# RagnarGrootKoerkamp/astar-pairwise-aligner

Hardware: AMD Instinct MI355X
Metric: DP cell-updates/sec (GCUPS), full bit-parallel DP, 100kbp@5% div (higher is better)
Workload: dtype u32

## Files before the change

### astar-pairwise-aligner_amd/capi.py

```python
from __future__ import annotations

import ctypes as C
import os
from pathlib import Path

import numpy as np

from . import _build

U64P = C.POINTER(C.c_uint64)

EXPORTED_SYMBOLS = [
    "astarpa2_simple", "astarpa2_full", "astarpa", "astarpa_gcsh", "astarpa_free_cigar",
    "pa_last_error", "pa_device_count", "pa_set_device",
    "pa_bp_profile_build", "pa_bp_compute", "pa_bp_fill", "pa_search", "pa_search_trace",
    "pa_batch_create", "pa_batch_run", "pa_batch_stats", "pa_batch_shape", "pa_batch_destroy",
    "pa_batch_create_banded", "pa_batch_create_trace", "pa_batch_align", "pa_batch_align_view", "pa_batch_trace_fallbacks", "pa_params_batch_align",
    "pa_pairs_read", "pa_pairs_count", "pa_pairs_get", "pa_pairs_free", "pa_write_results_csv", "pa_align_file",
    "pa_align", "pa_batch_align_multi", "pa_batch_create_trace_params",
    "pa_bp_ctx_create", "pa_bp_ctx_compute", "pa_bp_ctx_fill", "pa_bp_ctx_destroy",
    "pa_batch_create_params", "pa_batch_pair_stats", "pa_runtime_hints", "pa_batch_align_multi_params", "pa_release_pools", "pa_align_file_params", "pa_batch_params_supported", "pa_alloc_cache_stats", "pa_free_cigars",
    "pa_batch_full_info", "pa_batch_rdv_stats", "pa_combine_stats", "pa_params_nw", "pa_params_simple", "pa_params_full", "pa_debug_gcsh_probe", "pa_debug_gcsh_matches", "pa_debug_strip", "pa_batch_window_retries", "pa_batch_window_retry_bytes",
    "pa_batch_slice_info", "pa_set_reference_cost_only",
    "pa_search_batch_create", "pa_search_batch_run", "pa_search_batch_rows", "pa_search_batch_trace", "pa_search_batch_info",
    "pa_search_batch_destroy",
    "pa_affine_batch_create", "pa_affine_batch_run", "pa_affine_batch_align", "pa_affine_batch_info", "pa_affine_batch_destroy",
]

_lib = None


class PaError(RuntimeError):
    pass


def load(build_if_stale: bool = True) -> C.CDLL:
    global _lib
    if _lib is not None:
        return _lib
    path = _build.LIB_PATH
    if os.environ.get("PA_LIB_PATH"):
        from pathlib import Path

        path, build_if_stale = Path(os.environ["PA_LIB_PATH"]).resolve(), False
    if build_if_stale and _build.is_stale():
        try:
            _build.build()
        except Exception as e:
            if not path.exists():
                raise PaError(f"cannot build {path.name}: {e}") from e
    if not path.exists():
        raise PaError(f"{path} is missing: run __graft_entry__.build() (hipcc --offload-arch=gfx950)")
    L = C.CDLL(str(path))
    L.pa_runtime_hints.restype = C.c_int
    if hasattr(L, "pa_set_reference_cost_only"):
        L.pa_set_reference_cost_only.argtypes = [C.c_int]
        L.pa_set_reference_cost_only.restype = None
    L.pa_release_pools.restype = None
    L.pa_alloc_cache_stats.argtypes = [C.POINTER(C.c_uint64)] * 3
    L.pa_free_cigars.argtypes = [C.c_void_p, C.c_size_t]
    L.pa_free_cigars.restype = None
    L.pa_batch_params_supported.argtypes = [C.c_void_p]
    L.pa_batch_params_supported.restype = C.c_int
    L.pa_alloc_cache_stats.restype = None
    L.pa_runtime_hints()
    vp, sz = C.c_void_p, C.c_size_t
    L.pa_last_error.restype = C.c_char_p
    L.pa_device_count.restype = C.c_int
    L.pa_set_device.argtypes = [C.c_int]
    L.pa_bp_profile_build.argtypes = [vp, sz, vp, sz, vp, vp]
    L.pa_bp_profile_build.restype = C.c_int
    L.pa_bp_compute.argtypes = [vp, sz, vp, sz, vp, vp, C.c_int]
    L.pa_bp_compute.restype = C.c_int32
    L.pa_bp_fill.argtypes = [vp, sz, vp, sz, vp, vp, vp]
    L.pa_bp_fill.restype = C.c_int32
    L.pa_search.argtypes = [vp, sz, vp, sz, C.c_float, vp]
    L.pa_search.restype = C.c_int
    L.pa_search_trace.argtypes = [vp, sz, vp, sz, C.c_float, sz, C.POINTER(vp), C.POINTER(vp), C.POINTER(sz)]
    L.pa_search_trace.restype = C.c_int
    L.pa_search_batch_create.argtypes = [vp, vp, sz, vp, vp, sz, vp, vp, sz, C.c_float]
    L.pa_search_batch_create.restype = vp
    L.pa_search_batch_run.argtypes = [vp, vp, vp, C.POINTER(C.c_float)]
    L.pa_search_batch_rows.argtypes = [vp, vp, vp]
    L.pa_search_batch_trace.argtypes = [vp, vp, vp, vp]
    L.pa_search_batch_info.argtypes = [vp] + [C.POINTER(C.c_double)] * 4
    L.pa_search_batch_info.restype = None
    L.pa_search_batch_destroy.argtypes = [vp]
    L.pa_affine_batch_create.argtypes = [vp, vp, vp, vp, sz, vp, C.c_int]
    L.pa_affine_batch_create.restype = vp
    L.pa_affine_batch_run.argtypes = [vp, vp, C.POINTER(C.c_float)]
    L.pa_affine_batch_align.argtypes = [vp, vp, vp, C.POINTER(C.c_float), C.POINTER(C.c_float)]
    L.pa_affine_batch_info.argtypes = [vp] + [C.POINTER(C.c_double)] * 5
    L.pa_affine_batch_info.restype = None
    L.pa_affine_batch_destroy.argtypes = [vp]
    L.pa_search_batch_destroy.restype = None
    L.pa_batch_create.argtypes = [vp, vp, vp, vp, sz]
    L.pa_batch_create.restype = vp
    L.pa_batch_run.argtypes = [vp, vp, C.POINTER(C.c_float)]
    L.pa_batch_run.restype = C.c_int
    L.pa_batch_stats.argtypes = [vp] + [C.POINTER(C.c_double)] * 4
    L.pa_batch_full_info.argtypes = [vp] + [C.POINTER(C.c_double)] * 4 + [C.POINTER(C.c_double)]
    L.pa_batch_full_info.restype = None
    L.pa_batch_rdv_stats.argtypes = [vp, C.POINTER(C.c_uint64)]
    L.pa_combine_stats.argtypes = [C.POINTER(C.c_uint64), C.POINTER(C.c_uint64)]
    L.pa_combine_stats.restype = None
    L.pa_batch_rdv_stats.restype = C.c_int
    L.pa_batch_shape.argtypes = [vp, C.POINTER(C.c_int), C.POINTER(C.c_int), C.POINTER(C.c_double)]
    L.pa_batch_slice_info.argtypes = [vp] + [C.POINTER(C.c_double)] * 5
    L.pa_batch_slice_info.restype = C.c_int
    L.pa_batch_destroy.argtypes = [vp]
    L.pa_batch_create_banded.argtypes = [vp, vp, vp, vp, sz, C.c_float]
    L.pa_batch_create_banded.restype = vp
    L.pa_batch_create_trace.argtypes = [vp, vp, vp, vp, sz]
    L.pa_batch_create_trace.restype = vp
    L.pa_bp_ctx_create.argtypes = [vp, sz, vp, sz]
    L.pa_bp_ctx_create.restype = vp
    L.pa_bp_ctx_compute.argtypes = [vp, C.c_int32, C.c_int32, sz, sz, vp, C.c_int, C.POINTER(C.c_int32)]
    L.pa_bp_ctx_compute.restype = C.c_int
    L.pa_bp_ctx_fill.argtypes = [vp, C.c_int32, C.c_int32, sz, sz, vp, vp, vp]
    L.pa_bp_ctx_fill.restype = C.c_int
    L.pa_bp_ctx_destroy.argtypes = [vp]
    L.pa_batch_create_trace_params.argtypes = [vp, vp, vp, vp, sz, vp]
    L.pa_batch_create_trace_params.restype = vp
    L.pa_batch_create_params.argtypes = [vp, vp, vp, vp, sz, vp]
    L.pa_batch_create_params.restype = vp
    L.pa_batch_pair_stats.argtypes = [vp, vp]
    L.pa_batch_pair_stats.restype = C.c_int
    L.pa_batch_align.argtypes = [vp, vp, vp, C.POINTER(C.c_float), C.POINTER(C.c_float)]
    L.pa_batch_align.restype = C.c_int
    L.pa_batch_align_view.argtypes = [vp, vp, vp, vp, C.POINTER(C.c_float), C.POINTER(C.c_float)]
    L.pa_batch_align_view.restype = C.c_int
    L.pa_batch_trace_fallbacks.argtypes = [vp]
    L.pa_batch_trace_fallbacks.restype = C.c_size_t
    L.pa_batch_window_retries.argtypes = [vp]
    L.pa_batch_window_retries.restype = C.c_size_t
    L.pa_pairs_read.argtypes = [C.c_char_p]
    L.pa_pairs_read.restype = vp
    L.pa_pairs_count.argtypes = [vp]
    L.pa_pairs_count.restype = sz
    L.pa_pairs_get.argtypes = [vp, sz, C.POINTER(vp), C.POINTER(sz), C.POINTER(vp), C.POINTER(sz)]
    L.pa_pairs_get.restype = C.c_int
    L.pa_pairs_free.argtypes = [vp]
    L.pa_write_results_csv.argtypes = [C.c_char_p, vp, vp, sz]
    L.pa_write_results_csv.restype = C.c_int
    L.pa_batch_align_multi.argtypes = [vp, vp, vp, vp, sz, C.POINTER(C.c_int), C.c_int, vp, vp]
    L.pa_batch_align_multi.restype = C.c_int
    L.pa_batch_align_multi_params.argtypes = [vp, vp, vp, vp, sz, C.POINTER(C.c_int), C.c_int, vp, vp, vp, vp]
    L.pa_batch_align_multi_params.restype = C.c_int
    L.pa_align_file.argtypes = [C.c_char_p, C.c_char_p, C.POINTER(sz)]
    L.pa_align_file.restype = C.c_int
    L.pa_align_file_params.argtypes = [C.c_char_p, C.c_char_p, vp, C.POINTER(sz)]
    L.pa_align_file_params.restype = C.c_int
    for name in ("astarpa2_simple", "astarpa2_full", "astarpa"):
        if hasattr(L, name):
            f = getattr(L, name)
            f.argtypes = [vp, sz, vp, sz, C.POINTER(vp), C.POINTER(sz)]
            f.restype = C.c_uint64
    if hasattr(L, "astarpa_gcsh"):
        L.astarpa_gcsh.argtypes = [vp, sz, vp, sz, sz, sz, C.c_bool, C.POINTER(vp), C.POINTER(sz)]
        L.astarpa_gcsh.restype = C.c_uint64
    if hasattr(L, "astarpa_free_cigar"):
        L.astarpa_free_cigar.argtypes = [vp]
    _lib = L
    return L


def last_error() -> str:
    return (load().pa_last_error() or b"").decode()


def _p(arr: np.ndarray):
    return arr.ctypes.data_as(C.c_void_p)


def _buf(b: bytes):
    return C.cast(C.c_char_p(b), C.c_void_p)
# ... 669 lines not shown
```

### astar-pairwise-aligner_amd/csrc/slice_kernel.hpp

```cpp
#pragma once
#include <hip/hip_runtime.h>
#include <stdint.h>

namespace pa {
namespace slice {

#ifndef PA_SLICE_CLOCK_TURNS
#define PA_SLICE_CLOCK_TURNS 15
#endif
#ifndef PA_SLICE_YIELD
#define PA_SLICE_YIELD 2
#endif
constexpr int kPad = 64;
constexpr int kErrSpin = 7;
constexpr uint32_t kSpinLimit = 1u << 22;

struct SliceGroup {
    uint64_t a_off;
    uint64_t b_off;
    uint64_t h_off;
    uint32_t h_stride;
    int32_t n;
    int32_t nstrips;
    int32_t npairs;
    uint32_t first_pos;
    uint32_t ev_first, ev_count;
    uint32_t pad_;
};
struct SliceEvent {
    int32_t col;
    uint32_t mask;
};
struct SliceJob {
    uint32_t group, strip;
};
struct SlicePair {
    uint64_t code_off, prof_off;
    int32_t n, m;
    uint32_t pair;
    uint32_t pad_;
};

typedef uint32_t pa_slice_u32x2 __attribute__((ext_vector_type(2)));
__device__ __forceinline__ uint32_t dpp_wave_shr1(uint32_t old_, uint32_t src) {
    return (uint32_t)__builtin_amdgcn_update_dpp((int)old_, (int)src, 0x138, 0xf, 0xf, false);
}
__device__ __forceinline__ uint32_t dpp_wave_rol1(uint32_t x) {
    return (uint32_t)__builtin_amdgcn_update_dpp((int)x, (int)x, 0x134, 0xf, 0xf, false);
}
__device__ __forceinline__ uint2 ld_boundary(const uint2* p) {
    const unsigned long long v = __hip_atomic_load((const unsigned long long*)p, __ATOMIC_RELAXED, __HIP_MEMORY_SCOPE_AGENT);
    return make_uint2((uint32_t)v, (uint32_t)(v >> 32));
}
__device__ __forceinline__ void st_boundary(uint2* p, uint32_t hp, uint32_t hm) {
    __hip_atomic_store((unsigned long long*)p, (unsigned long long)hp | ((unsigned long long)hm << 32), __ATOMIC_RELAXED, __HIP_MEMORY_SCOPE_AGENT);
}

#define PA_SLICE_ROW_PAIR(vpA, vmA, vpB, vmB, nb0A, nb1A, nb0B, nb1B, a0, a1, hpp, hmp, hpo, hmo)                                      \
    do {                                                                                                                                \
        uint32_t zA_, zB_, hmA_, hpA_;                                                                                                  \
        asm volatile(                                                                                                                   \
            "v_xor_b32 %[zA], %[a1_], %[nb1A_]\n\t"                                                                                     \
            "v_xor_b32 %[zB], %[a1_], %[nb1B_]\n\t"                                                                                     \
            "v_bitop3_b32 %[zA], %[a0_], %[nb0A_], %[zA] bitop3:0x28\n\t"                                                               \
            "v_bitop3_b32 %[zB], %[a0_], %[nb0B_], %[zB] bitop3:0x28\n\t"                                                               \
            "v_bitop3_b32 %[zA], %[zA], %[vmA_], %[hmp_] bitop3:0xfe\n\t"                                                               \
            "v_and_b32 %[hmA], %[zA], %[vpA_]\n\t"                                                                                      \
            "v_bitop3_b32 %[hpA], %[vmA_], %[zA], %[vpA_] bitop3:0xf1\n\t"                                                              \
            "v_bitop3_b32 %[zB], %[zB], %[vmB_], %[hmA] bitop3:0xfe\n\t"                                                                \
            "v_bitop3_b32 %[vpA_], %[hmp_], %[zA], %[hpp_] bitop3:0xf1\n\t"                                                             \
            "v_and_b32 %[hmB], %[zB], %[vpB_]\n\t"                                                                                      \
            "v_and_b32 %[vmA_], %[hpp_], %[zA]\n\t"                                                                                     \
            "v_bitop3_b32 %[hpB], %[vmB_], %[zB], %[vpB_] bitop3:0xf1\n\t"                                                              \
            "v_bitop3_b32 %[vpB_], %[hmA], %[zB], %[hpA] bitop3:0xf1\n\t"                                                               \
            "v_and_b32 %[vmB_], %[hpA], %[zB]"                                                                                          \
            : [zA] "=&v"(zA_), [zB] "=&v"(zB_), [hmA] "=&v"(hmA_), [hpA] "=&v"(hpA_), [hmB] "=&v"(hmo), [hpB] "=&v"(hpo),              \
              [vpA_] "+v"(vpA), [vmA_] "+v"(vmA), [vpB_] "+v"(vpB), [vmB_] "+v"(vmB)                                                    \
            : [a0_] "v"(a0), [a1_] "v"(a1), [nb0A_] "v"(nb0A), [nb1A_] "v"(nb1A), [nb0B_] "v"(nb0B), [nb1B_] "v"(nb1B), [hpp_] "v"(hpp), \
              [hmp_] "v"(hmp));                                                                                                         \
    } while (0)

template <int R>
__global__ __launch_bounds__(64, 2) void slice_kernel(const SliceJob* __restrict__ jobs, int njobs, const SliceGroup* __restrict__ groups,
                                                      const SliceEvent* __restrict__ events, const uint2* __restrict__ A, const uint2* __restrict__ B,
                                                      uint2* H, uint2* V, uint32_t* ticket_err, unsigned long long* dbg) {
    static_assert(R % 2 == 0, "rows are stepped in pairs");
    const int lane = (int)threadIdx.x;
    const uint32_t wave_slot = (uint32_t)__builtin_amdgcn_s_getreg((4 - 1) << 11 | 4) & 15u;
    for (;;) {
        uint32_t tk = 0;
        if (lane == 0) tk = atomicAdd(ticket_err, 1u);
        tk = (uint32_t)__builtin_amdgcn_readfirstlane((int)tk);
        if (tk >= (uint32_t)njobs) break;
        const SliceJob job = jobs[tk];
        const SliceGroup grp = groups[job.group];
        const unsigned long long t_job0 = dbg ? __builtin_amdgcn_s_memrealtime() : 0ull;
        unsigned long long t_parked = 0, n_parks = 0;
        [[maybe_unused]] bool waited_before = false;
        [[maybe_unused]] int slack = 0;
        const int s = (int)job.strip, n = grp.n;
        const bool has_in = s > 0, has_out = s + 1 < grp.nstrips;
        const uint2* Ag = A + grp.a_off + kPad;
        const size_t row0 = grp.b_off + ((size_t)s * 64 + (size_t)lane) * R;
        const uint2* Hin = H + grp.h_off + (size_t)(has_in ? s - 1 : 0) * grp.h_stride + kPad;
        uint2* Hout = H + grp.h_off + (size_t)(has_out ? s : 0) * grp.h_stride + kPad;
        const SliceEvent* ev = events + grp.ev_first;
        uint32_t nb0[R], nb1[R], vp[R], vm[R];
#pragma unroll
        for (int i = 0; i < R; ++i) {
            const uint2 b = B[row0 + i];
            nb0[i] = b.x;
            nb1[i] = b.y;
            vp[i] = ~0u;
            vm[i] = 0u;
        }
        constexpr int kWaitStep = 8;
        uint32_t o_hp = 0, o_hm = 0, o_a0 = 0, o_a1 = 0;
        uint32_t ev_i = 0;
        int ev_col = ev[0].col;
        const int nchunks = (n + 63 + 63) / 64;
        const __amdgpu_buffer_rsrc_t hrs = __builtin_amdgcn_make_buffer_rsrc((void*)Hout, 0, (int)((uint32_t)n * 8u), 0x00020000);
        unsigned long long nA = 0, nH = ~0ull;
        uint2 kA = Ag[lane], kH = make_uint2(~0u, 0u);
        if (has_in) kH = ld_boundary(Hin + lane);
        __builtin_amdgcn_s_waitcnt(0);
        for (int q = 0; q < nchunks; ++q) {
#if PA_SLICE_CLOCK_TURNS
            if ((((uint32_t)__builtin_amdgcn_s_memrealtime() >> PA_SLICE_CLOCK_TURNS) ^ wave_slot) & 1u) __builtin_amdgcn_s_setprio(1);
            else __builtin_amdgcn_s_setprio(0);
#else
            if (((uint32_t)q ^ wave_slot) & 1u) __builtin_amdgcn_s_setprio(1);
            else __builtin_amdgcn_s_setprio(0);
#endif
            uint2 cA = kA, cH = kH;
            const int col = q * 64 + lane;
            if (has_in) {
                uint32_t spins = 0;
                const unsigned long long t_p0 = dbg ? __builtin_amdgcn_s_memrealtime() : 0ull;
                while (col < n && (cH.x & cH.y) != 0u) {
                    __builtin_amdgcn_s_sleep(32);
                    cH = ld_boundary(Hin + col);
                    if (++spins > kSpinLimit) {
                        atomicCAS(ticket_err + 1, 0u, (uint32_t)kErrSpin);
                        cH = make_uint2(~0u, 0u);
                    }
                }
                const bool waited = __builtin_amdgcn_readfirstlane((int)(__ballot(spins != 0u) != 0ull)) != 0;
#if PA_SLICE_YIELD == 1
                if (waited) __builtin_amdgcn_s_setprio(0);
#elif PA_SLICE_YIELD == 2
                if (waited || waited_before) __builtin_amdgcn_s_setprio(0);
                waited_before = waited;
#elif PA_SLICE_YIELD >= 3
                slack = waited ? PA_SLICE_YIELD : (slack > 0 ? slack - 1 : 0);
                if (slack > 0) __builtin_amdgcn_s_setprio(0);
#endif
                if (dbg && waited) {
                    t_parked += __builtin_amdgcn_s_memrealtime() - t_p0;
                    n_parks += 1;
                }
            }
            const int pcol = min(col + 64, n + kPad - 1);
            const bool more = q + 1 < nchunks;
            if (more) {
                asm volatile("global_load_dwordx2 %0, %1, off ; pa_prefetch_load" : "=v"(nA) : "v"(Ag + pcol) : "memory");
                if (has_in) asm volatile("global_load_dwordx2 %0, %1, off sc1 ; pa_prefetch_load" : "=v"(nH) : "v"(Hin + pcol) : "memory");
            }
            const int jend = min(64, n + 63 - q * 64);
            const int wait_at = more ? kWaitStep : -1;
            for (int j = 0; j < jend; ++j) {
                if (j == wait_at) {
                    asm volatile("s_waitcnt vmcnt(8) ; pa_prefetch_wait" : "+v"(nA), "+v"(nH)::"memory");
                    kA = make_uint2((uint32_t)nA, (uint32_t)(nA >> 32));
                    if (has_in) kH = make_uint2((uint32_t)nH, (uint32_t)(nH >> 32));
                }
                const int c = q * 64 + j - lane;
                const uint32_t a0 = dpp_wave_shr1(cA.x, o_a0), a1 = dpp_wave_shr1(cA.y, o_a1);
                uint32_t hpp = dpp_wave_shr1(cH.x, o_hp), hmp = dpp_wave_shr1(cH.y, o_hm);
                cA.x = dpp_wave_rol1(cA.x);
                cA.y = dpp_wave_rol1(cA.y);
                cH.x = dpp_wave_rol1(cH.x);
                cH.y = dpp_wave_rol1(cH.y);
                o_a0 = a0;
                o_a1 = a1;
                if ((unsigned)c < (unsigned)n) {
#pragma unroll
                    for (int i = 0; i < R; i += 2) {
                        uint32_t hpo, hmo;
                        PA_SLICE_ROW_PAIR(vp[i], vm[i], vp[i + 1], vm[i + 1], nb0[i], nb1[i], nb0[i + 1], nb1[i + 1], a0, a1, hpp, hmp, hpo, hmo);
                        hpp = hpo;
                        hmp = hmo;
                    }
                    o_hp = hpp;
                    o_hm = hmp;
                    {
                        const pa_slice_u32x2 d = {hpp, hmp};
                        __builtin_amdgcn_raw_buffer_store_b64(d, hrs, (lane == 63 && has_out) ? (uint32_t)c * 8u : 0x7FFFFFF0u, 0, 16);
                    }
                    if (c + 1 == ev_col) {
                        const uint32_t mask = ev[ev_i].mask;
#pragma unroll
                        for (int i = 0; i < R; ++i) {
                            atomicOr(&V[row0 + i].x, vp[i] & mask);
                            atomicOr(&V[row0 + i].y, vm[i] & mask);
                            asm volatile("" ::: "memory");
                        }
                        ++ev_i;
                        ev_col = ev_i < grp.ev_count ? ev[ev_i].col : -1;
                        __builtin_amdgcn_s_waitcnt(0);
                    }
                }
            }
        }
        if (dbg && lane == 0) {
            const unsigned long long dt = __builtin_amdgcn_s_memrealtime() - t_job0;
            atomicMin(dbg + 0, dt);
            atomicMax(dbg + 1, dt);
            atomicAdd(dbg + 2, dt);
            atomicAdd(dbg + 3, 1ull);
            atomicAdd(dbg + 4, t_parked);
            atomicAdd(dbg + 5, n_parks);
            if (s == 0) {
                atomicMin(dbg + 6, dt);
                atomicMax(dbg + 7, dt);
            }
            const uint32_t xcc = (uint32_t)__builtin_amdgcn_s_getreg((4 - 1) << 11 | 20) & 7u;
            atomicAdd(dbg + 8 + 2 * xcc, dt - t_parked);
            atomicAdd(dbg + 9 + 2 * xcc, 1ull);
        }
    }
}


__global__ __launch_bounds__(256) void slice_pack_a_kernel(const SliceGroup* __restrict__ groups, const SlicePair* __restrict__ spairs,
                                                           const uint32_t* __restrict__ codes, uint2* __restrict__ A) {
    const SliceGroup grp = groups[blockIdx.x];
    const int lane = (int)(threadIdx.x & 63), q = (int)(blockIdx.y * 4 + (threadIdx.x >> 6));
    if (q * 32 >= grp.n) return;
    const int p = lane & 31, half = lane >> 5, word = 2 * q + half;
    uint32_t w = 0;
    if (p < grp.npairs) {
        const SlicePair sp = spairs[grp.first_pos + p];
        if (word < (sp.n + 15) / 16) w = codes[sp.code_off + word];
    }
    uint32_t a0 = 0, a1 = 0;
#pragma unroll
    for (int k = 0; k < 16; ++k) {
        const unsigned long long b0 = __ballot((w >> (2 * k)) & 1u), b1 = __ballot((w >> (2 * k + 1)) & 1u);
        if ((lane & 15) == k) {
            a0 = (lane & 16) ? (uint32_t)(b0 >> 32) : (uint32_t)b0;
            a1 = (lane & 16) ? (uint32_t)(b1 >> 32) : (uint32_t)b1;
        }
    }
    const int c = q * 32 + lane;
    if (lane < 32 && c < grp.n) A[grp.a_off + kPad + c] = make_uint2(a0, a1);
}

__global__ __launch_bounds__(256) void slice_pack_b_kernel(const SliceGroup* __restrict__ groups, const SlicePair* __restrict__ spairs,
                                                           const uint64_t* __restrict__ prof, uint2* __restrict__ B, int rows_per_strip) {
    const SliceGroup grp = groups[blockIdx.x];
    const int lane = (int)(threadIdx.x & 63), j = (int)(blockIdx.y * 4 + (threadIdx.x >> 6));
    if ((long long)j * 64 >= (long long)grp.nstrips * rows_per_strip) return;
    const int p = lane & 31, half = lane >> 5;
    uint32_t x0 = 0, x1 = 0;
    if (p < grp.npairs) {
        const SlicePair sp = spairs[grp.first_pos + p];
        if (j < (sp.m + 63) / 64) {
            const uint64_t p0 = prof[2 * (sp.prof_off + j)], p1 = prof[2 * (sp.prof_off + j) + 1];
            x0 = (uint32_t)(p0 >> (32 * half));
            x1 = (uint32_t)(p1 >> (32 * half));
        }
    }
    uint32_t nb0 = 0, nb1 = 0;
#pragma unroll
    for (int k = 0; k < 32; ++k) {
        const unsigned long long b0 = __ballot((x0 >> k) & 1u), b1 = __ballot((x1 >> k) & 1u);
        if ((lane & 31) == k) {
            nb0 = half ? (uint32_t)(b0 >> 32) : (uint32_t)b0;
            nb1 = half ? (uint32_t)(b1 >> 32) : (uint32_t)b1;
        }
    }
    B[grp.b_off + (size_t)j * 64 + lane] = make_uint2(nb0, nb1);
}

constexpr int kScoreSpan = 4096;
__global__ __launch_bounds__(64) void slice_score_kernel(const SliceGroup* __restrict__ groups, const SlicePair* __restrict__ spairs,
                                                         const uint2* __restrict__ V, int32_t* __restrict__ cost_out) {
    const SliceGroup grp = groups[blockIdx.x];
    const int lane = (int)threadIdx.x;
    int my_m = 0, my_n = 0;
    uint32_t my_pair = 0;
    if (lane < grp.npairs) {
        const SlicePair sp = spairs[grp.first_pos + lane];
        my_m = sp.m;
        my_n = sp.n;
        my_pair = sp.pair;
    }
    int max_m = my_m;
#pragma unroll
    for (int o = 32; o > 0; o >>= 1) max_m = max(max_m, __shfl_xor(max_m, o));
    const int lo = (int)blockIdx.y * kScoreSpan, hi = min(max_m, lo + kScoreSpan);
    if (lo >= max_m) return;
    int acc = blockIdx.y == 0 ? my_n : 0;
    for (int r0 = lo; r0 < hi; r0 += 64) {
        const int r = r0 + lane;
        uint2 v = make_uint2(0u, 0u);
        if (r < hi) v = V[grp.b_off + r];
        for (int p = 0; p < grp.npairs; ++p) {
            const int mp = __shfl(my_m, p);
            const bool in = r < mp;
            const int pos = __popcll(__ballot(in && ((v.x >> p) & 1u))), neg = __popcll(__ballot(in && ((v.y >> p) & 1u)));
            if (lane == p) acc += pos - neg;
        }
    }
    if (lane < grp.npairs && acc != 0) atomicAdd(&cost_out[my_pair], acc);
}

}
}
```

### astar-pairwise-aligner_amd/csrc/slice_plan.hpp

```cpp
#pragma once
#include <hip/hip_runtime.h>

#include <cstddef>
#include <cstdint>

namespace pa {
namespace slice {

struct Plan;

constexpr int kRowsPerLane[] = {52, 50, 48, 46, 44, 42, 40, 36, 32, 28};

int choose_rows_per_lane(const size_t* a_len, const size_t* b_len, size_t pairs, double simds, double* est_ns);

Plan* create(const size_t* a_len, const size_t* b_len, size_t pairs, const size_t* code_off, const size_t* prof_off, int rows_per_lane);
void destroy(Plan* p);

int run(Plan* p, hipStream_t s, const uint32_t* d_codes, const uint64_t* d_prof, int32_t* d_costs, uint32_t* d_ticket_err, hipEvent_t ev0, hipEvent_t ev1);

struct Info {
    int rows_per_lane;
    size_t groups, jobs;
    double valu_instructions;
    double computed_rows_cells;
    double device_bytes;
    double boundary_bytes;
};
Info info(const Plan* p);
constexpr int kStepOverheadInstr = 24;

}
}
```

### astar-pairwise-aligner_amd/csrc/slice_unit.hip

```cpp
#include "slice_plan.hpp"

#include <algorithm>
#include <cmath>
#include <cstdio>
#include <cstdlib>
#include <memory>
#include <numeric>
#include <vector>

#include "pa_hip_internal.hpp"
#include "slice_kernel.hpp"

namespace pa {
namespace slice {

struct Plan {
    int R = 52;
    size_t pairs = 0;
    std::vector<SliceGroup> groups;
    std::vector<SliceJob> jobs;
    size_t a_elems = 0, b_elems = 0, h_elems = 0;
    unsigned max_col_blocks = 0, max_row_blocks = 0;
    double valu = 0, computed = 0;
    DeviceBuf d_groups, d_events, d_jobs, d_spairs, d_A, d_B, d_V, d_H;
};

static int strips_for(size_t m, int R) { return (int)((m + (size_t)64 * R - 1) / ((size_t)64 * R)); }

static constexpr double kNsPerRowStep = 16.2, kNsStepOverhead = 53.7, kChainPenalty = 0.0015;

int choose_rows_per_lane(const size_t* a_len, const size_t* b_len, size_t pairs, double simds, double* est_ns) {
    if (const char* e = getenv("PA_SLICE")) {
        if (atoi(e) == 0) return 0;
    }
    size_t live = 0;
    for (size_t i = 0; i < pairs; ++i) {
        live += a_len[i] > 0 && b_len[i] > 0;
        if (a_len[i] >= (size_t(1) << 27) || b_len[i] >= (size_t(1) << 27)) return 0;
    }
    const bool forced = getenv("PA_SLICE") && atoi(getenv("PA_SLICE")) > 0;
    if (live < 64 && !forced) return 0;
    std::vector<uint32_t> order;
    for (size_t i = 0; i < pairs; ++i)
        if (a_len[i] > 0 && b_len[i] > 0) order.push_back((uint32_t)i);
    std::sort(order.begin(), order.end(), [&](uint32_t x, uint32_t y) { return a_len[x] != a_len[y] ? a_len[x] < a_len[y] : (b_len[x] != b_len[y] ? b_len[x] < b_len[y] : x < y); });
    int best_r = 0;
    double best = -1;
    const double slots = simds * 2.0;
    for (const int R : kRowsPerLane) {
        if (forced && atoi(getenv("PA_SLICE")) > 1 && atoi(getenv("PA_SLICE")) != R) continue;
        double work = 0, longest = 0, jobs = 0;
        for (size_t g = 0; g * 32 < order.size(); ++g) {
            size_t n = 0, m = 0;
            for (size_t t = g * 32; t < std::min(order.size(), g * 32 + 32); ++t) {
                n = std::max(n, a_len[order[t]]);
                m = std::max(m, b_len[order[t]]);
            }
            const int S = strips_for(m, R);
            const double per_strip = ((double)n + 63.0) * (R * kNsPerRowStep + kNsStepOverhead) * (1.0 + kChainPenalty * (S - 1));
            work += per_strip * S;
            jobs += S;
            longest = std::max(longest, per_strip + 128.0 * (S - 1) * (R * kNsPerRowStep + kNsStepOverhead));
        }
        const double waves = std::min(jobs, slots);
        const double speed = waves <= simds ? 1.165 : 1.0 + 0.165 * (slots - waves) / simds;
        const double rounds = jobs > slots ? std::ceil(jobs / slots) * (work / jobs) : work / waves;
        const double t = std::max(longest / 1.165, rounds / speed);
        if (best < 0 || t < best) {
            best = t;
            best_r = R;
        }
    }
    if (est_ns) *est_ns = best;
    return best_r;
}

Plan* create(const size_t* a_len, const size_t* b_len, size_t pairs, const size_t* code_off, const size_t* prof_off, int rows_per_lane) {
    auto p = std::make_unique<Plan>();
    p->R = rows_per_lane;
    p->pairs = pairs;
    const int R = rows_per_lane;
    std::vector<uint32_t> order;
    for (size_t i = 0; i < pairs; ++i)
        if (a_len[i] > 0 && b_len[i] > 0) order.push_back((uint32_t)i);
    std::sort(order.begin(), order.end(), [&](uint32_t x, uint32_t y) { return a_len[x] != a_len[y] ? a_len[x] < a_len[y] : (b_len[x] != b_len[y] ? b_len[x] < b_len[y] : x < y); });
    std::vector<SlicePair> spairs(order.size());
    std::vector<SliceEvent> events;
    size_t a_at = 0, b_at = 0, h_at = 0;
    size_t max_n = 0, max_rows = 0;
    const size_t ngroups = (order.size() + 31) / 32;
    for (size_t gi = 0; gi < ngroups; ++gi) {
        const size_t g = ngroups - 1 - gi;
        SliceGroup grp{};
        grp.first_pos = (uint32_t)(g * 32);
        grp.npairs = (int32_t)std::min<size_t>(32, order.size() - g * 32);
        size_t n = 0, m = 0;
        for (int t = 0; t < grp.npairs; ++t) {
            const uint32_t i = order[g * 32 + t];
            n = std::max(n, a_len[i]);
            m = std::max(m, b_len[i]);
            spairs[g * 32 + t] = SlicePair{(uint64_t)code_off[i], (uint64_t)prof_off[i], (int32_t)a_len[i], (int32_t)b_len[i], i, 0u};
        }
        grp.n = (int32_t)n;
        grp.nstrips = strips_for(m, R);
        grp.a_off = a_at;
        grp.b_off = b_at;
        grp.h_off = h_at;
        grp.h_stride = (uint32_t)(n + 2 * kPad);
        a_at += n + 2 * kPad;
        b_at += (size_t)grp.nstrips * 64 * R;
        h_at += (size_t)(grp.nstrips - 1) * grp.h_stride;
        grp.ev_first = (uint32_t)events.size();
        for (int t = 0; t < grp.npairs; ++t) {
            const int32_t col = (int32_t)a_len[order[g * 32 + t]];
            if (events.size() > grp.ev_first && events.back().col == col) events.back().mask |= 1u << t;
            else events.push_back(SliceEvent{col, 1u << t});
        }
        grp.ev_count = (uint32_t)events.size() - grp.ev_first;
        max_n = std::max(max_n, n);
        max_rows = std::max(max_rows, (size_t)grp.nstrips * 64 * R);
        for (int s = 0; s < grp.nstrips; ++s) p->jobs.push_back(SliceJob{(uint32_t)p->groups.size(), (uint32_t)s});
        p->valu += (double)grp.nstrips * ((double)n + 63.0) * (7.0 * R + kStepOverheadInstr);
        p->computed += (double)grp.nstrips * 64.0 * R * (double)n * 32.0;
        p->groups.push_back(grp);
    }
    p->a_elems = a_at;
    p->b_elems = b_at;
    p->h_elems = h_at;
    p->max_col_blocks = (unsigned)((max_n + 127) / 128);
    p->max_row_blocks = (unsigned)((max_rows / 64 + 3) / 4);
    if (p->groups.empty()) return p.release();
    if (events.empty()) events.push_back(SliceEvent{0, 0});
    if (!p->d_groups.alloc(p->groups.size() * sizeof(SliceGroup)) || !p->d_events.alloc(events.size() * sizeof(SliceEvent)) ||
        !p->d_jobs.alloc(p->jobs.size() * sizeof(SliceJob)) || !p->d_spairs.alloc(spairs.size() * sizeof(SlicePair)) || !p->d_A.alloc(a_at * 8) ||
        !p->d_B.alloc(b_at * 8) || !p->d_V.alloc(b_at * 8) || !p->d_H.alloc(std::max<size_t>(h_at, 8) * 8))
        return nullptr;
    if (!hip_ok(hipMemcpy(p->d_groups.ptr, p->groups.data(), p->groups.size() * sizeof(SliceGroup), hipMemcpyHostToDevice), "H2D slice groups") ||
        !hip_ok(hipMemcpy(p->d_events.ptr, events.data(), events.size() * sizeof(SliceEvent), hipMemcpyHostToDevice), "H2D slice events") ||
        !hip_ok(hipMemcpy(p->d_jobs.ptr, p->jobs.data(), p->jobs.size() * sizeof(SliceJob), hipMemcpyHostToDevice), "H2D slice jobs") ||
        !hip_ok(hipMemcpy(p->d_spairs.ptr, spairs.data(), spairs.size() * sizeof(SlicePair), hipMemcpyHostToDevice), "H2D slice pairs") ||
        !hip_ok(hipMemset(p->d_A.ptr, 0, a_at * 8), "memset slice A"))
        return nullptr;
    return p.release();
}

void destroy(Plan* p) { delete p; }

template <int R>
static hipError_t launch_slice(int grid, hipStream_t s, const Plan* p, uint32_t* d_ticket_err, unsigned long long* dbg) {
    hipLaunchKernelGGL((slice_kernel<R>), dim3((unsigned)grid), dim3(64), 0, s, p->d_jobs.as<SliceJob>(), (int)p->jobs.size(), p->d_groups.as<SliceGroup>(),
                       p->d_events.as<SliceEvent>(), p->d_A.as<uint2>(), p->d_B.as<uint2>(), p->d_H.as<uint2>(), p->d_V.as<uint2>(), d_ticket_err, dbg);
    return hipGetLastError();
}

int run(Plan* p, hipStream_t s, const uint32_t* d_codes, const uint64_t* d_prof, int32_t* d_costs, uint32_t* d_ticket_err, hipEvent_t ev0, hipEvent_t ev1) {
    if (!hip_ok(hipMemsetAsync(d_ticket_err, 0, 8, s), "memset slice ticket")) return PA_E_HIP;
    if (p->groups.empty()) {
        if (ev0 && (!hip_ok(hipEventRecord(ev0, s), "event") || !hip_ok(hipEventRecord(ev1, s), "event"))) return PA_E_HIP;
        return 0;
    }
    const unsigned G = (unsigned)p->groups.size();
    hipLaunchKernelGGL(slice_pack_a_kernel, dim3(G, p->max_col_blocks), dim3(256), 0, s, p->d_groups.as<SliceGroup>(), p->d_spairs.as<SlicePair>(), d_codes,
                       p->d_A.as<uint2>());
    hipLaunchKernelGGL(slice_pack_b_kernel, dim3(G, p->max_row_blocks), dim3(256), 0, s, p->d_groups.as<SliceGroup>(), p->d_spairs.as<SlicePair>(), d_prof,
                       p->d_B.as<uint2>(), 64 * p->R);
    if (!hip_ok(hipGetLastError(), "slice transposes")) return PA_E_HIP;
    if (!hip_ok(hipMemsetAsync(p->d_V.ptr, 0, p->b_elems * 8, s), "memset slice V")) return PA_E_HIP;
    if (p->h_elems && !hip_ok(hipMemsetAsync(p->d_H.ptr, 0xFF, p->h_elems * 8, s), "memset slice boundaries")) return PA_E_HIP;
    int cus = 256;
    {
        int dev = 0;
        hipDeviceProp_t prop;
        if (hipGetDevice(&dev) == hipSuccess && hipGetDeviceProperties(&prop, dev) == hipSuccess && prop.multiProcessorCount > 0) cus = prop.multiProcessorCount;
    }
    const int grid = (int)std::min<size_t>(p->jobs.size(), (size_t)cus * 8);
    static const bool jobtimes = getenv("PA_SLICE_JOBTIMES") != nullptr;
    unsigned long long* dbg = nullptr;
    if (jobtimes && hipMalloc((void**)&dbg, 192) == hipSuccess) {
        const unsigned long long init[24] = {~0ull, 0, 0, 0, 0, 0, ~0ull, 0};
        if (hipMemcpyAsync(dbg, init, 192, hipMemcpyHostToDevice, s) != hipSuccess || hipStreamSynchronize(s) != hipSuccess) dbg = nullptr;
    }
    if (ev0 && !hip_ok(hipEventRecord(ev0, s), "event")) return PA_E_HIP;
    hipError_t e = hipSuccess;
    switch (p->R) {
        case 52: e = launch_slice<52>(grid, s, p, d_ticket_err, dbg); break;
        case 50: e = launch_slice<50>(grid, s, p, d_ticket_err, dbg); break;
        case 48: e = launch_slice<48>(grid, s, p, d_ticket_err, dbg); break;
        case 46: e = launch_slice<46>(grid, s, p, d_ticket_err, dbg); break;
        case 44: e = launch_slice<44>(grid, s, p, d_ticket_err, dbg); break;
        case 42: e = launch_slice<42>(grid, s, p, d_ticket_err, dbg); break;
        case 40: e = launch_slice<40>(grid, s, p, d_ticket_err, dbg); break;
        case 36: e = launch_slice<36>(grid, s, p, d_ticket_err, dbg); break;
        case 32: e = launch_slice<32>(grid, s, p, d_ticket_err, dbg); break;
        case 28: e = launch_slice<28>(grid, s, p, d_ticket_err, dbg); break;
        default: set_error("slice: no kernel for %d rows per lane", p->R); return PA_E_INTERNAL;
    }
    if (!hip_ok(e, "slice_kernel")) return PA_E_HIP;
    if (ev1 && !hip_ok(hipEventRecord(ev1, s), "event")) return PA_E_HIP;
    if (dbg) {
        unsigned long long h[24] = {0};
        if (hipMemcpyAsync(h, dbg, 192, hipMemcpyDeviceToHost, s) == hipSuccess && hipStreamSynchronize(s) == hipSuccess && h[3]) {
            std::fprintf(stderr, "[slice jobs] awake us per job by XCD:");
            for (int x = 0; x < 8; ++x) std::fprintf(stderr, " %d: %.0f (%llu)", x, h[9 + 2 * x] ? h[8 + 2 * x] * 0.01 / (double)h[9 + 2 * x] : 0.0, h[9 + 2 * x]);
            std::fprintf(stderr, "\n");
            std::fprintf(stderr, "[slice jobs] R %d: %llu jobs, us per job: min %.1f mean %.1f max %.1f (first strips: min %.1f max %.1f); asleep behind the strip above: %.2f %% of the job time, %.1f waits per job\n",
                         p->R, h[3], h[0] * 0.01, h[2] * 0.01 / (double)h[3], h[1] * 0.01, h[6] * 0.01, h[7] * 0.01, 100.0 * (double)h[4] / (double)h[2], (double)h[5] / (double)h[3]);
        }
        (void)hipFree(dbg);
    }
    hipLaunchKernelGGL(slice_score_kernel, dim3(G, (p->max_row_blocks * 256u + kScoreSpan - 1) / kScoreSpan), dim3(64), 0, s, p->d_groups.as<SliceGroup>(), p->d_spairs.as<SlicePair>(), p->d_V.as<uint2>(), d_costs);
    if (!hip_ok(hipGetLastError(), "slice_score_kernel")) return PA_E_HIP;
    return 0;
}

Info info(const Plan* p) {
    Info i{};
    i.rows_per_lane = p->R;
    i.groups = p->groups.size();
    i.jobs = p->jobs.size();
    i.valu_instructions = p->valu;
    i.computed_rows_cells = p->computed;
    i.device_bytes = (double)(p->a_elems + 2 * p->b_elems + p->h_elems) * 8.0;
    i.boundary_bytes = (double)p->h_elems * 8.0;
    return i;
}

}
}
```

### include/pa_bitpacking_hip.h

```cpp
#ifndef PA_BITPACKING_HIP_H
#define PA_BITPACKING_HIP_H

#include <stddef.h>
#include <stdint.h>

#ifdef __cplusplus
extern "C" {
#endif

#define PA_E_INVALID_BASE (-1)
#define PA_E_HIP (-2)
#define PA_E_TIMEOUT (-3)
#define PA_E_ARG (-4)
#define PA_E_INTERNAL (-5)
#define PA_E_NOMEM (-6)

const char* pa_last_error(void);

int pa_device_count(void);
int pa_set_device(int device);

int pa_bp_profile_build(const uint8_t* a, size_t n, const uint8_t* b, size_t m, uint64_t* a2, uint64_t* b2);

int32_t pa_bp_compute(const uint64_t* a2, size_t n, const uint64_t* b2, size_t w, uint64_t* h2, uint64_t* v2,
                      int exact_end);

int32_t pa_bp_fill(const uint64_t* a2, size_t n, const uint64_t* b2, size_t w, uint64_t* h2, uint64_t* v2,
                   uint64_t* values);

typedef struct pa_bp_ctx pa_bp_ctx;
pa_bp_ctx* pa_bp_ctx_create(const uint8_t* a, size_t n, const uint8_t* b, size_t m);
int pa_bp_ctx_compute(pa_bp_ctx* ctx, int32_t i0, int32_t i1, size_t w0, size_t w1, uint64_t* v, int h_mode, int32_t* sum_out);
int pa_bp_ctx_fill(pa_bp_ctx* ctx, int32_t i0, int32_t i1, size_t w0, size_t w1, uint64_t* v, uint64_t* values, int8_t* h_bottom);
void pa_bp_ctx_destroy(pa_bp_ctx* ctx);

int pa_search(const uint8_t* pattern, size_t plen, const uint8_t* text, size_t tlen, float unmatched_cost, int32_t* out);
int pa_search_trace(const uint8_t* pattern, size_t plen, const uint8_t* text, size_t tlen, float unmatched_cost, size_t idx,
                    char** cigar_out, int32_t** path_out, size_t* npos_out);

typedef struct pa_search_batch pa_search_batch;
pa_search_batch* pa_search_batch_create(const uint8_t* const* patterns, const size_t* plens, size_t npatterns,
                                        const uint8_t* const* texts, const size_t* tlens, size_t ntexts,
                                        const uint32_t* q_pattern, const uint32_t* q_text, size_t nqueries,
                                        float unmatched_cost);
int pa_search_batch_run(pa_search_batch* sb, int32_t* best_cost, uint64_t* best_idx, float* kernel_ms);
int pa_search_batch_rows(const pa_search_batch* sb, int32_t* out, const uint64_t* offsets);
int pa_search_batch_trace(pa_search_batch* sb, const uint64_t* idx, char** cigars_out, int64_t* start_out);
void pa_search_batch_info(const pa_search_batch* sb, double* waves, double* packed, double* chained, double* lane_use);
void pa_search_batch_destroy(pa_search_batch* sb);
typedef struct pa_batch pa_batch;

pa_batch* pa_batch_create(const uint8_t* const* a, const size_t* a_len, const uint8_t* const* b,
                          const size_t* b_len, size_t pairs);
pa_batch* pa_batch_create_banded(const uint8_t* const* a, const size_t* a_len, const uint8_t* const* b,
                                 const size_t* b_len, size_t pairs, float divergence_hint);
int pa_batch_run(pa_batch* plan, int32_t* cost_out, float* kernel_ms);
void pa_batch_stats(const pa_batch* plan, double* cells, double* word_updates, double* strips, double* algo_bytes);
void pa_batch_shape(const pa_batch* plan, int* k, int* sequential, double* valu_instructions);
int pa_batch_slice_info(const pa_batch* plan, double* groups, double* jobs, double* computed_cells, double* device_bytes, double* boundary_bytes);
void pa_batch_destroy(pa_batch* plan);

pa_batch* pa_batch_create_trace(const uint8_t* const* a, const size_t* a_len, const uint8_t* const* b,
                                const size_t* b_len, size_t pairs);
struct pa_astarpa2_params;
pa_batch* pa_batch_create_trace_params(const uint8_t* const* a, const size_t* a_len, const uint8_t* const* b, const size_t* b_len,
                                       size_t pairs, const struct pa_astarpa2_params* trace_params);
int pa_batch_align(pa_batch* plan, int32_t* cost_out, char** cigar_out, float* forward_ms, float* trace_ms);
int pa_batch_align_view(pa_batch* plan, int32_t* cost_out, const char** text_out, uint32_t* text_len_out, float* forward_ms, float* trace_ms);
void pa_free_cigars(char** cigars, size_t n);
size_t pa_batch_trace_fallbacks(const pa_batch* plan);
size_t pa_batch_window_retries(const pa_batch* plan);
double pa_batch_window_retry_bytes(const pa_batch* plan);

struct pa_astarpa2_stats;
pa_batch* pa_batch_create_params(const uint8_t* const* a, const size_t* a_len, const uint8_t* const* b, const size_t* b_len,
                                 size_t pairs, const struct pa_astarpa2_params* params);
int pa_batch_pair_stats(const pa_batch* plan, struct pa_astarpa2_stats* stats_out);
int pa_batch_params_supported(const struct pa_astarpa2_params* params);
void pa_batch_full_info(const pa_batch* plan, double* build_ms, double* matches, double* probes, double* rounds, double* phase_wave_ms);
int pa_batch_rdv_stats(const pa_batch* plan, uint64_t* out4);
long pa_debug_gcsh_matches(const uint8_t* a, size_t a_len, const uint8_t* b, size_t b_len, int32_t k, int32_t p_local, int32_t* out_ij, size_t cap_out);
int pa_debug_gcsh_probe(const uint8_t* a, size_t a_len, const uint8_t* b, size_t b_len, int32_t k, int32_t p_local, const int32_t* queries,
                        size_t nq, int32_t* out);
typedef struct pa_strip_probe_job {
    const uint8_t* a;
    size_t a_len;
    const uint8_t* b;
    size_t b_len;
    int32_t col0, n, word0, nlanes, tap, fill_word0, fill_stride, hin_is_hout;
    uint32_t* v;
    const uint8_t* hin;
    const uint32_t* values;
    uint8_t* hout;
    int32_t sum;
} pa_strip_probe_job;
int pa_debug_strip(int mode, int variant, int nwaves, uint32_t patience, pa_strip_probe_job* jobs, size_t njobs, uint64_t* counters4);

int pa_batch_align_multi(const uint8_t* const* a, const size_t* a_len, const uint8_t* const* b, const size_t* b_len, size_t pairs,
                         const int* devices, int ndevices, int32_t* cost_out, char** cigar_out);
int pa_batch_align_multi_params(const uint8_t* const* a, const size_t* a_len, const uint8_t* const* b, const size_t* b_len, size_t pairs,
                                const int* devices, int ndevices, const struct pa_astarpa2_params* params, int32_t* cost_out,
                                char** cigar_out, struct pa_astarpa2_stats* stats_out);

typedef struct pa_pairs pa_pairs;
pa_pairs* pa_pairs_read(const char* path);
size_t pa_pairs_count(const pa_pairs* pairs);
int pa_pairs_get(const pa_pairs* pairs, size_t i, const uint8_t** a, size_t* a_len, const uint8_t** b, size_t* b_len);
void pa_pairs_free(pa_pairs* pairs);
int pa_write_results_csv(const char* path, const int32_t* costs, const char* const* cigars, size_t n);
int pa_align_file(const char* input_path, const char* output_path, size_t* pairs_out);
struct pa_astarpa2_params;
int pa_align_file_params(const char* input_path, const char* output_path, const struct pa_astarpa2_params* params, size_t* pairs_out);

#ifdef __cplusplus
}
#endif
#endif
```

Measured before the change: 232,000.

## Trim per-column step overhead in slice kernel and allow odd rows-per-lane

Rewrites the inner column loop of the slice kernel around a uniform step counter. The A character now shifts in through a DPP shift plus a lane-0 select, the H store offset is an incrementing register, the column-bounds check only runs at the edges, and event capture is gated by a scalar threshold. This is meant to cut the per-step scalar and vector overhead. It also adds odd row counts per lane (51, 49, ...) with a single-row tail macro. The planner gains these candidates and a lower overhead constant, which gives finer load balance across SIMDs but costs more template instantiations and more complex edge handling.

```diff
diff --git a/astar-pairwise-aligner_amd/capi.py b/astar-pairwise-aligner_amd/capi.py
--- a/astar-pairwise-aligner_amd/capi.py
+++ b/astar-pairwise-aligner_amd/capi.py
@@ -21,7 +21,7 @@
     "pa_bp_ctx_create", "pa_bp_ctx_compute", "pa_bp_ctx_fill", "pa_bp_ctx_destroy",
     "pa_batch_create_params", "pa_batch_pair_stats", "pa_runtime_hints", "pa_batch_align_multi_params", "pa_release_pools", "pa_align_file_params", "pa_batch_params_supported", "pa_alloc_cache_stats", "pa_free_cigars",
     "pa_batch_full_info", "pa_batch_rdv_stats", "pa_combine_stats", "pa_params_nw", "pa_params_simple", "pa_params_full", "pa_debug_gcsh_probe", "pa_debug_gcsh_matches", "pa_debug_strip", "pa_batch_window_retries", "pa_batch_window_retry_bytes",
-    "pa_batch_slice_info", "pa_set_reference_cost_only",
+    "pa_batch_slice_info", "pa_slice_choose_rows", "pa_set_reference_cost_only",
     "pa_search_batch_create", "pa_search_batch_run", "pa_search_batch_rows", "pa_search_batch_trace", "pa_search_batch_info",
     "pa_search_batch_destroy",
     "pa_affine_batch_create", "pa_affine_batch_run", "pa_affine_batch_align", "pa_affine_batch_info", "pa_affine_batch_destroy",
diff --git a/astar-pairwise-aligner_amd/csrc/slice_kernel.hpp b/astar-pairwise-aligner_amd/csrc/slice_kernel.hpp
--- a/astar-pairwise-aligner_amd/csrc/slice_kernel.hpp
+++ b/astar-pairwise-aligner_amd/csrc/slice_kernel.hpp
@@ -80,11 +80,26 @@
               [hmp_] "v"(hmp));                                                                                                         \
     } while (0)
 
+#define PA_SLICE_ROW_ONE(vpA, vmA, nb0A, nb1A, a0, a1, hpp, hmp, hpo, hmo)                                                              \
+    do {                                                                                                                                \
+        uint32_t zA_;                                                                                                                   \
+        asm volatile(                                                                                                                   \
+            "v_xor_b32 %[zA], %[a1_], %[nb1A_]\n\t"                                                                                     \
+            "v_bitop3_b32 %[zA], %[a0_], %[nb0A_], %[zA] bitop3:0x28\n\t"                                                               \
+            "v_bitop3_b32 %[zA], %[zA], %[vmA_], %[hmp_] bitop3:0xfe\n\t"                                                               \
+            "v_and_b32 %[hmA], %[zA], %[vpA_]\n\t"                                                                                      \
+            "v_bitop3_b32 %[hpA], %[vmA_], %[zA], %[vpA_] bitop3:0xf1\n\t"                                                              \
+            "v_bitop3_b32 %[vpA_], %[hmp_], %[zA], %[hpp_] bitop3:0xf1\n\t"                                                             \
+            "v_and_b32 %[vmA_], %[hpp_], %[zA]"                                                                                         \
+            : [zA] "=&v"(zA_), [hmA] "=&v"(hmo), [hpA] "=&v"(hpo), [vpA_] "+v"(vpA), [vmA_] "+v"(vmA)                                   \
+            : [a0_] "v"(a0), [a1_] "v"(a1), [nb0A_] "v"(nb0A), [nb1A_] "v"(nb1A), [hpp_] "v"(hpp), [hmp_] "v"(hmp));                    \
+    } while (0)
+
 template <int R>
 __global__ __launch_bounds__(64, 2) void slice_kernel(const SliceJob* __restrict__ jobs, int njobs, const SliceGroup* __restrict__ groups,
                                                       const SliceEvent* __restrict__ events, const uint2* __restrict__ A, const uint2* __restrict__ B,
                                                       uint2* H, uint2* V, uint32_t* ticket_err, unsigned long long* dbg) {
-    static_assert(R % 2 == 0, "rows are stepped in pairs");
+    static_assert(R >= 2, "rows are stepped in pairs; an odd R ends with a single row");
     const int lane = (int)threadIdx.x;
     const uint32_t wave_slot = (uint32_t)__builtin_amdgcn_s_getreg((4 - 1) << 11 | 4) & 15u;
     for (;;) {
@@ -115,13 +130,36 @@
             vm[i] = 0u;
         }
         constexpr int kWaitStep = 8;
-        uint32_t o_hp = 0, o_hm = 0, o_a0 = 0, o_a1 = 0;
+        const int n_u = __builtin_amdgcn_readfirstlane(n);
+        uint32_t o_hp = 0, o_hm = 0, a0 = 0, a1 = 0;
+        uint32_t lane0 = lane == 0 ? ~0u : 0u;
+        asm volatile("" : "+v"(lane0));
         uint32_t ev_i = 0;
-        int ev_col = ev[0].col;
-        const int nchunks = (n + 63 + 63) / 64;
-        const __amdgpu_buffer_rsrc_t hrs = __builtin_amdgcn_make_buffer_rsrc((void*)Hout, 0, (int)((uint32_t)n * 8u), 0x00020000);
+        uint32_t ev_t = (uint32_t)ev[0].col + (uint32_t)lane;
+        uint32_t cap_from = (uint32_t)__builtin_amdgcn_readlane((int)ev_t, 63) - 63u;
+        const auto capture = [&](uint32_t t) __attribute__((always_inline)) {
+            asm volatile("; pa_step_capture" ::: "memory");
+            if (t == ev_t) {
+                const uint32_t mask = ev[ev_i].mask;
+#pragma unroll
+                for (int i = 0; i < R; ++i) {
+                    atomicOr(&V[row0 + i].x, vp[i] & mask);
+                    atomicOr(&V[row0 + i].y, vm[i] & mask);
+                    asm volatile("" ::: "memory");
+                }
+                ++ev_i;
+                ev_t = ev_i < grp.ev_count ? (uint32_t)ev[ev_i].col + (uint32_t)lane : ~0u;
+                __builtin_amdgcn_s_waitcnt(0);
+            }
+            cap_from = (uint32_t)__builtin_amdgcn_readlane((int)ev_t, 63) - 63u;
+        };
+        const int nchunks = (n_u + 63 + 63) / 64;
+        const __amdgpu_buffer_rsrc_t hrs = __builtin_amdgcn_make_buffer_rsrc((void*)Hout, 0, (int)((uint32_t)n_u * 8u), 0x00020000);
+        uint32_t st_off = (lane == 63 && has_out) ? 0u - 8u * 63u : (uint32_t)n_u * 8u;
+        const uint32_t all_from = 63u, all_count = (uint32_t)max(n_u - 63, 0);
         unsigned long long nA = 0, nH = ~0ull;
-        uint2 kA = Ag[lane], kH = make_uint2(~0u, 0u);
+        const int lane_a = (lane - 1) & 63;
+        uint2 kA = Ag[lane_a], kH = make_uint2(~0u, 0u);
         if (has_in) kH = ld_boundary(Hin + lane);
         __builtin_amdgcn_s_waitcnt(0);
         for (int q = 0; q < nchunks; ++q) {
@@ -161,33 +199,47 @@
                 }
             }
             const int pcol = min(col + 64, n + kPad - 1);
+            const int pcol_a = min(q * 64 + lane_a + 64, n + kPad - 1);
             const bool more = q + 1 < nchunks;
             if (more) {
-                asm volatile("global_load_dwordx2 %0, %1, off ; pa_prefetch_load" : "=v"(nA) : "v"(Ag + pcol) : "memory");
+                asm volatile("global_load_dwordx2 %0, %1, off ; pa_prefetch_load" : "=v"(nA) : "v"(Ag + pcol_a) : "memory");
                 if (has_in) asm volatile("global_load_dwordx2 %0, %1, off sc1 ; pa_prefetch_load" : "=v"(nH) : "v"(Hin + pcol) : "memory");
             }
-            const int jend = min(64, n + 63 - q * 64);
-            const int wait_at = more ? kWaitStep : -1;
-            for (int j = 0; j < jend; ++j) {
-                if (j == wait_at) {
+            const uint32_t t0 = (uint32_t)__builtin_amdgcn_readfirstlane(q * 64);
+            const uint32_t tend = t0 + (uint32_t)__builtin_amdgcn_readfirstlane(min(64, n_u + 63 - q * 64));
+            const uint32_t wait_at = more ? t0 + (uint32_t)kWaitStep : ~0u;
+            for (uint32_t t = t0; t != tend; ++t) {
+                if (__builtin_expect(t >= cap_from, 0)) capture(t);
+                if (__builtin_expect(t == wait_at, 0)) {
                     asm volatile("s_waitcnt vmcnt(8) ; pa_prefetch_wait" : "+v"(nA), "+v"(nH)::"memory");
                     kA = make_uint2((uint32_t)nA, (uint32_t)(nA >> 32));
                     if (has_in) kH = make_uint2((uint32_t)nH, (uint32_t)(nH >> 32));
                 }
-                const int c = q * 64 + j - lane;
-                const uint32_t a0 = dpp_wave_shr1(cA.x, o_a0), a1 = dpp_wave_shr1(cA.y, o_a1);
-                uint32_t hpp = dpp_wave_shr1(cH.x, o_hp), hmp = dpp_wave_shr1(cH.y, o_hm);
                 cA.x = dpp_wave_rol1(cA.x);
                 cA.y = dpp_wave_rol1(cA.y);
+                a0 = dpp_wave_shr1(a0, a0);
+                a1 = dpp_wave_shr1(a1, a1);
+                a0 = (uint32_t)__builtin_amdgcn_bitop3_b32((int)a0, (int)cA.x, (int)lane0, 0xd8);
+                a1 = (uint32_t)__builtin_amdgcn_bitop3_b32((int)a1, (int)cA.y, (int)lane0, 0xd8);
+                uint32_t hpp = dpp_wave_shr1(cH.x, o_hp), hmp = dpp_wave_shr1(cH.y, o_hm);
                 cH.x = dpp_wave_rol1(cH.x);
                 cH.y = dpp_wave_rol1(cH.y);
-                o_a0 = a0;
-                o_a1 = a1;
-                if ((unsigned)c < (unsigned)n) {
-#pragma unroll
-                    for (int i = 0; i < R; i += 2) {
+                bool at_column = true;
+                if (__builtin_expect(t - all_from >= all_count, 0)) {
+                    asm volatile("; pa_step_edge" ::: "memory");
+                    at_column = t - (uint32_t)lane < (uint32_t)n_u;
+                }
+                if (at_column) {
+#pragma unroll
+                    for (int i = 0; i + 1 < R; i += 2) {
                         uint32_t hpo, hmo;
                         PA_SLICE_ROW_PAIR(vp[i], vm[i], vp[i + 1], vm[i + 1], nb0[i], nb1[i], nb0[i + 1], nb1[i + 1], a0, a1, hpp, hmp, hpo, hmo);
+                        hpp = hpo;
+                        hmp = hmo;
+                    }
+                    if constexpr (R % 2 != 0) {
+                        uint32_t hpo, hmo;
+                        PA_SLICE_ROW_ONE(vp[R - 1], vm[R - 1], nb0[R - 1], nb1[R - 1], a0, a1, hpp, hmp, hpo, hmo);
                         hpp = hpo;
                         hmp = hmo;
                     }
@@ -195,23 +247,13 @@
                     o_hm = hmp;
                     {
                         const pa_slice_u32x2 d = {hpp, hmp};
-                        __builtin_amdgcn_raw_buffer_store_b64(d, hrs, (lane == 63 && has_out) ? (uint32_t)c * 8u : 0x7FFFFFF0u, 0, 16);
+                        __builtin_amdgcn_raw_buffer_store_b64(d, hrs, st_off, 0, 16);
                     }
-                    if (c + 1 == ev_col) {
-                        const uint32_t mask = ev[ev_i].mask;
-#pragma unroll
-                        for (int i = 0; i < R; ++i) {
-                            atomicOr(&V[row0 + i].x, vp[i] & mask);
-                            atomicOr(&V[row0 + i].y, vm[i] & mask);
-                            asm volatile("" ::: "memory");
-                        }
-                        ++ev_i;
-                        ev_col = ev_i < grp.ev_count ? ev[ev_i].col : -1;
-                        __builtin_amdgcn_s_waitcnt(0);
-                    }
-                }
-            }
-        }
+                }
+                st_off += 8u;
+            }
+        }
+        capture((uint32_t)n_u + 63u);
         if (dbg && lane == 0) {
             const unsigned long long dt = __builtin_amdgcn_s_memrealtime() - t_job0;
             atomicMin(dbg + 0, dt);
diff --git a/astar-pairwise-aligner_amd/csrc/slice_plan.hpp b/astar-pairwise-aligner_amd/csrc/slice_plan.hpp
--- a/astar-pairwise-aligner_amd/csrc/slice_plan.hpp
+++ b/astar-pairwise-aligner_amd/csrc/slice_plan.hpp
@@ -9,7 +9,7 @@
 
 struct Plan;
 
-constexpr int kRowsPerLane[] = {52, 50, 48, 46, 44, 42, 40, 36, 32, 28};
+constexpr int kRowsPerLane[] = {52, 51, 50, 49, 48, 47, 46, 45, 44, 43, 42, 41, 40, 36, 32, 28};
 
 int choose_rows_per_lane(const size_t* a_len, const size_t* b_len, size_t pairs, double simds, double* est_ns);
 
@@ -27,7 +27,7 @@
     double boundary_bytes;
 };
 Info info(const Plan* p);
-constexpr int kStepOverheadInstr = 24;
+constexpr int kStepOverheadInstr = 13;
 
 }
 }
diff --git a/astar-pairwise-aligner_amd/csrc/slice_unit.hip b/astar-pairwise-aligner_amd/csrc/slice_unit.hip
--- a/astar-pairwise-aligner_amd/csrc/slice_unit.hip
+++ b/astar-pairwise-aligner_amd/csrc/slice_unit.hip
@@ -49,6 +49,7 @@
     const double slots = simds * 2.0;
     for (const int R : kRowsPerLane) {
         if (forced && atoi(getenv("PA_SLICE")) > 1 && atoi(getenv("PA_SLICE")) != R) continue;
+        const bool pinned = forced && atoi(getenv("PA_SLICE")) == R;
         double work = 0, longest = 0, jobs = 0;
         for (size_t g = 0; g * 32 < order.size(); ++g) {
             size_t n = 0, m = 0;
@@ -62,6 +63,7 @@
             jobs += S;
             longest = std::max(longest, per_strip + 128.0 * (S - 1) * (R * kNsPerRowStep + kNsStepOverhead));
         }
+        if (R % 2 != 0 && jobs < slots && !pinned) continue;
         const double waves = std::min(jobs, slots);
         const double speed = waves <= simds ? 1.165 : 1.0 + 0.165 * (slots - waves) / simds;
         const double rounds = jobs > slots ? std::ceil(jobs / slots) * (work / jobs) : work / waves;
@@ -184,11 +186,17 @@
     hipError_t e = hipSuccess;
     switch (p->R) {
         case 52: e = launch_slice<52>(grid, s, p, d_ticket_err, dbg); break;
+        case 51: e = launch_slice<51>(grid, s, p, d_ticket_err, dbg); break;
         case 50: e = launch_slice<50>(grid, s, p, d_ticket_err, dbg); break;
+        case 49: e = launch_slice<49>(grid, s, p, d_ticket_err, dbg); break;
         case 48: e = launch_slice<48>(grid, s, p, d_ticket_err, dbg); break;
+        case 47: e = launch_slice<47>(grid, s, p, d_ticket_err, dbg); break;
         case 46: e = launch_slice<46>(grid, s, p, d_ticket_err, dbg); break;
+        case 45: e = launch_slice<45>(grid, s, p, d_ticket_err, dbg); break;
         case 44: e = launch_slice<44>(grid, s, p, d_ticket_err, dbg); break;
+        case 43: e = launch_slice<43>(grid, s, p, d_ticket_err, dbg); break;
         case 42: e = launch_slice<42>(grid, s, p, d_ticket_err, dbg); break;
+        case 41: e = launch_slice<41>(grid, s, p, d_ticket_err, dbg); break;
         case 40: e = launch_slice<40>(grid, s, p, d_ticket_err, dbg); break;
         case 36: e = launch_slice<36>(grid, s, p, d_ticket_err, dbg); break;
         case 32: e = launch_slice<32>(grid, s, p, d_ticket_err, dbg); break;
@@ -227,3 +235,7 @@
 
 }
 }
+
+extern "C" int pa_slice_choose_rows(const size_t* a_len, const size_t* b_len, size_t pairs, double simds, double* est_ns) {
+    return pa::slice::choose_rows_per_lane(a_len, b_len, pairs, simds, est_ns);
+}
diff --git a/include/pa_bitpacking_hip.h b/include/pa_bitpacking_hip.h
--- a/include/pa_bitpacking_hip.h
+++ b/include/pa_bitpacking_hip.h
@@ -58,6 +58,7 @@
 void pa_batch_stats(const pa_batch* plan, double* cells, double* word_updates, double* strips, double* algo_bytes);
 void pa_batch_shape(const pa_batch* plan, int* k, int* sequential, double* valu_instructions);
 int pa_batch_slice_info(const pa_batch* plan, double* groups, double* jobs, double* computed_cells, double* device_bytes, double* boundary_bytes);
+int pa_slice_choose_rows(const size_t* a_len, const size_t* b_len, size_t pairs, double simds, double* est_ns);
 void pa_batch_destroy(pa_batch* plan);
 
 pa_batch* pa_batch_create_trace(const uint8_t* const* a, const size_t* a_len, const uint8_t* const* b,
```

After: 234,100 (median of 6 runs). No clear change (+0.9%).
